# felipemcoelho/nf4-triton-dequantization

Hardware: AMD Instinct MI355X
Metric: dequantized elements/s (4096x4096 NF4->bf16, blocksize 64 / nested 256) (higher is better)
Workload: dtype f32

## Files before the change

nf4_triton_dequantization_amd/csrc/nf4_dequant.hip:

```cpp
#include <hip/hip_runtime.h>
#include <stdint.h>

#include <type_traits>

#include "../../include/nf4_dequant.h"
#include "nf4_common.h"
#include "nf4_dequant_plan.h"

namespace {

using namespace nf4dq;

#if NF4_FLAT_STAMPS
#define NF4_FSTAMP(slot_, val_)                                                                      \
    do {                                                                                             \
        __builtin_amdgcn_sched_barrier(0);                                                           \
        if (lane == 0) stamps[(blockIdx.x * kFlatWaves + (threadIdx.x >> 6)) * 4u + (slot_)] = (val_);    \
        __builtin_amdgcn_sched_barrier(0);                                                           \
    } while (0)
#define NF4_FNOW() __builtin_amdgcn_s_memrealtime()
#else
#define NF4_FSTAMP(slot_, val_) \
    do {                        \
    } while (0)
#define NF4_FNOW() 0ull
#endif

#ifndef NF4_DQ_AUX_STORE
#define NF4_DQ_AUX_STORE 18
#endif
#ifndef NF4_DQ_AUX_LOAD
#define NF4_DQ_AUX_LOAD 2
#endif
#ifndef NF4_DQ_SCALE_FIRST
#define NF4_DQ_SCALE_FIRST 0
#endif
#ifndef NF4_DQ_SCALE_NT
#define NF4_DQ_SCALE_NT 0
#endif
#ifndef NF4_DQ_DECODE
#define NF4_DQ_DECODE 1
#endif
#ifndef NF4_DQ_SINGLE_FAST
#define NF4_DQ_SINGLE_FAST 1
#endif
#ifndef NF4_DQ_ABL_NOSCALE
#define NF4_DQ_ABL_NOSCALE 0
#endif

constexpr int kAuxStore = NF4_DQ_AUX_STORE;
constexpr int kAuxLoad = NF4_DQ_AUX_LOAD;

struct TileIn {
    uint32_t w[kU];
    uint32_t a1;
    float a2;
};

template <int DT>
__device__ __forceinline__ uint32_t tile_block(const Desc& D, uint32_t base, uint32_t lane) {
    constexpr uint32_t kTileBytes = tile_bytes<DT>();
    const uint32_t bsh = D.blk_shift;
    const uint32_t bpt = kTileBytes >> bsh;
    uint32_t g = (base >> bsh) + (bpt ? (lane & (bpt - 1u)) : 0u);
    const uint32_t nblk = (D.nbytes + (1u << bsh) - 1u) >> bsh;
    g = g < nblk ? g : nblk - 1u;
    return g + D.blk_base;
}

template <int DT, int MODE, bool FENCE = false>
__device__ __forceinline__ TileIn tile_load(const Desc& D, __amdgpu_buffer_rsrc_t rp, uint32_t base, uint32_t lane) {
    constexpr uint32_t LB = lane_bytes<DT>();
    TileIn in;
    auto packed_loads = [&]() {
#pragma unroll
        for (int j = 0; j < kU; ++j) {
            const uint32_t off = base + 64u * LB * j + LB * lane;
            if constexpr (LB == 4) {
                in.w[j] = __builtin_amdgcn_raw_buffer_load_b32(rp, off, 0, kAuxLoad);
            } else {
                in.w[j] = __builtin_amdgcn_raw_buffer_load_b16(rp, off, 0, kAuxLoad);
            }
        }
    };
    if constexpr (!NF4_DQ_SCALE_FIRST) {
        packed_loads();
        if constexpr (FENCE) __builtin_amdgcn_sched_barrier(0);
    }
    const uint32_t g = tile_block<DT>(D, base, lane);
    if constexpr (NF4_DQ_ABL_NOSCALE) {
        in.a1 = g & 255u;
        in.a2 = 0.01f;
    } else if constexpr (MODE == kRef) {
        const uint32_t r = fdiv(g, D.bpr);
        const uint32_t b = g - r * D.bpr.d;
        const uint8_t* pa1 = D.a1 + fmodu(g, D.nb);
        const float* pa2 = D.a2 + fmodu(r * D.groups + (b >> 2), D.n2);
        if constexpr (NF4_DQ_SCALE_NT) {
            in.a1 = __builtin_nontemporal_load(pa1);
            in.a2 = __builtin_nontemporal_load(pa2);
        } else {
            in.a1 = *pa1;
            in.a2 = *pa2;
        }
    } else if constexpr (MODE == kSingle) {
        const uint32_t r = fdiv(g, D.bpr);
        const uint32_t b = g - r * D.bpr.d;
        in.a2 = D.a2[r * D.n2.d + b];
    } else if constexpr (MODE == kBnb) {
        in.a1 = D.a1[g];
        in.a2 = D.a2[g >> D.blk2_shift];
    } else {
        in.a2 = D.a2[g];
    }
    if constexpr (NF4_DQ_SCALE_FIRST) packed_loads();
    return in;
}

template <int DT, int MODE>
__device__ __forceinline__ void tile_finish(const Desc& D, __amdgpu_buffer_rsrc_t ro, const float* lut,
                                            const TileIn& in, uint32_t base, uint32_t lane, const float* code2s) {
    float s;
    if constexpr (MODE == kRef) {
        s = ((float)in.a1 / 127.0f) * in.a2;
    } else if constexpr (MODE == kBnb) {
        s = code2s[in.a1] * in.a2 + D.offset;
    } else {
        s = in.a2;
    }
    const uint32_t bsh = D.blk_shift;
    constexpr uint32_t kOB = out_bytes_per_packed_byte<DT>();
    constexpr uint32_t LB = lane_bytes<DT>();
#pragma unroll
    for (int j = 0; j < kU; ++j) {
        const uint32_t rel = 64u * LB * j + LB * lane;
        const float sj = __shfl(s, (int)(rel >> bsh), 64);
        const uint32_t w = in.w[j];
        const uint32_t hi4 = (w >> 2) & 0x3C3C3C3Cu;
        const uint32_t lo4 = (w << 2) & 0x3C3C3C3Cu;
        const char* t = reinterpret_cast<const char*>(lut);
        float v[2 * LB];
#pragma unroll
        for (int k = 0; k < (int)LB; ++k) {
            v[2 * k] = *reinterpret_cast<const float*>(t + ((hi4 >> (8 * k)) & 0xFFu)) * sj;
            v[2 * k + 1] = *reinterpret_cast<const float*>(t + ((lo4 >> (8 * k)) & 0xFFu)) * sj;
        }
        const uint32_t ob = (base + rel) * kOB;
        if constexpr (DT == NF4DQ_F32) {
            u32x4 o = {__float_as_uint(v[0]), __float_as_uint(v[1]), __float_as_uint(v[2]), __float_as_uint(v[3])};
            __builtin_amdgcn_raw_buffer_store_b128(o, ro, ob, 0, kAuxStore);
        } else {
            u32x4 o = {pack2<DT>(v[0], v[1]), pack2<DT>(v[2], v[3]), pack2<DT>(v[4], v[5]), pack2<DT>(v[6], v[7])};
            __builtin_amdgcn_raw_buffer_store_b128(o, ro, ob, 0, kAuxStore);
        }
    }
}


struct TblCtx {
    char* tbl;
    uint32_t tb;
    f32x2 c01;
};

template <int DT, int MODE>
__device__ __forceinline__ void tile_finish_tbl(const Desc& D, __amdgpu_buffer_rsrc_t ro, const TileIn& in,
                                                uint32_t base, uint32_t lane, const float* code2s,
                                                const TblCtx& c) {
    float s;
    if constexpr (MODE == kRef) {
        s = ((float)in.a1 / 127.0f) * in.a2;
    } else if constexpr (MODE == kBnb) {
        s = code2s[in.a1] * in.a2 + D.offset;
    } else {
        s = in.a2;
    }
    const uint32_t bsh = D.blk_shift;
    const uint32_t k = lane & 7u;
#pragma unroll
    for (int j = 0; j < kU; ++j) {
        const uint32_t rel = 256u * j + 4u * lane;
        const float sj = __shfl(s, (int)(rel >> bsh), 64);
        block_table_write<DT>(c.tbl, c.tb, k, c.c01, sj);
        const u32x4 ov = block_table_decode(c.tbl, c.tb, in.w[j]);
        __builtin_amdgcn_raw_buffer_store_b128(ov, ro, (base + rel) * 4u, 0, kAuxStore);
    }
}

template <int MAXB>
__device__ __forceinline__ uint32_t find_matrix(const Batch<MAXB>& bt, uint32_t t, uint32_t k) {
    if constexpr (MAXB > 1) {
        while (k + 1 < bt.count && t >= bt.d[k + 1].tile_begin) ++k;
    }
    return k;
}

struct Cursor {
    uint32_t t, k, base;
    bool valid;
};

template <int DT, int MAXB>
__device__ __forceinline__ Cursor cursor_at(const Batch<MAXB>& bt, uint32_t t, uint32_t k_hint) {
    constexpr uint32_t kTileBytes = tile_bytes<DT>();
    Cursor c;
    c.t = t;
    c.valid = t < bt.total_tiles;
    c.k = c.valid ? find_matrix(bt, t, k_hint) : k_hint;
    c.base = c.valid ? (t - bt.d[c.k].tile_begin) * kTileBytes : 0xFFFFF000u;
    return c;
}

template <int DT, int MAXB>
__device__ __forceinline__ void make_rsrcs(const Batch<MAXB>& bt, uint32_t k, __amdgpu_buffer_rsrc_t& rp,
                                           __amdgpu_buffer_rsrc_t& ro) {
    constexpr uint32_t kOB = out_bytes_per_packed_byte<DT>();
    rp = __builtin_amdgcn_make_buffer_rsrc((void*)bt.d[k].packed, 0, bt.d[k].nbytes, kRsrcFlags);
    ro = __builtin_amdgcn_make_buffer_rsrc((void*)bt.d[k].out, 0, bt.d[k].nbytes * kOB, kRsrcFlags);
}

template <int DT, int MODE, int MAXB>
__global__ __launch_bounds__(kFlatWg) void nf4_flat_kernel(const Batch<MAXB> bt) {
    __shared__ __attribute__((aligned(16))) float lut[16];
    __shared__ __attribute__((aligned(16))) float code2s[MODE == kBnb ? 256 : 1];
    constexpr bool kTbl = NF4_DQ_DECODE == 1 && DT != NF4DQ_F32;
    __shared__ __attribute__((aligned(256))) char tbl[kTbl ? kFlatWaves * 2048 : 4];
    const uint32_t lane = threadIdx.x & 63u;
#if NF4_FLAT_STAMPS
    const unsigned long long t_entry = NF4_FNOW();
    unsigned long long tiles_done = 0;
    unsigned long long* const stamps = bt.stamps;
#endif
    const uint32_t t0 = __builtin_amdgcn_readfirstlane(blockIdx.x * kFlatWaves + (threadIdx.x >> 6));
    const uint32_t nwaves = gridDim.x * kFlatWaves;

    float c2w = 0.0f;
    if constexpr (MODE == kBnb) c2w = bt.d[0].code2[threadIdx.x & 255u];
    Cursor ca = cursor_at<DT>(bt, t0, 0u);
    __amdgpu_buffer_rsrc_t rpa, roa;
    make_rsrcs<DT>(bt, ca.k, rpa, roa);
    TileIn A = tile_load<DT, MODE>(bt.d[ca.k], rpa, ca.base, lane);
    const bool multi = !NF4_DQ_SINGLE_FAST || ca.t + nwaves < bt.total_tiles;
    if (multi) {
        const u32x4 z = {0u, 0u, 0u, 0u};
#pragma unroll
        for (int j = 0; j < kU; ++j) __builtin_amdgcn_raw_buffer_store_b128(z, roa, 0xFFFFF000u + 16u * j, 0, kAuxStore);
    }
    write_lut(lut);
    if constexpr (MODE == kBnb) {
        if constexpr (kFlatWg >= 256) {
            if (threadIdx.x < 256u) code2s[threadIdx.x] = c2w;
        } else {
            for (uint32_t i = threadIdx.x; i < 256u; i += kFlatWg) code2s[i] = bt.d[0].code2[i];
        }
    }
    __syncthreads();
    TblCtx tc{};
    if constexpr (kTbl) {
        tc.tbl = tbl;
        tc.tb = ((threadIdx.x >> 6) << 11) + ((lane >> 3) << 8);
        tc.c01 = *reinterpret_cast<const f32x2*>(lut + 2u * (lane & 7u));
    }
    if (!ca.valid) {
        NF4_FSTAMP(0, t_entry);
        NF4_FSTAMP(1, 0ull);
        NF4_FSTAMP(2, NF4_FNOW());
        NF4_FSTAMP(3, 0ull);
        return;
    }
    if (!multi) {
        if constexpr (kTbl) tile_finish_tbl<DT, MODE>(bt.d[ca.k], roa, A, ca.base, lane, code2s, tc);
        else tile_finish<DT, MODE>(bt.d[ca.k], roa, lut, A, ca.base, lane, code2s);
#if NF4_FLAT_STAMPS
        NF4_FSTAMP(1, NF4_FNOW());
        __builtin_amdgcn_s_waitcnt(0);
        NF4_FSTAMP(0, t_entry);
        NF4_FSTAMP(2, NF4_FNOW());
        NF4_FSTAMP(3, 1ull);
#endif
        return;
    }
    while (true) {
        const Cursor cb = cursor_at<DT>(bt, ca.t + nwaves, ca.k);
        __amdgpu_buffer_rsrc_t rpb = rpa, rob = roa;
        if (MAXB > 1 && cb.k != ca.k) make_rsrcs<DT>(bt, cb.k, rpb, rob);
        TileIn B = tile_load<DT, MODE>(bt.d[cb.k], rpb, cb.base, lane);
        if constexpr (kTbl) tile_finish_tbl<DT, MODE>(bt.d[ca.k], roa, A, ca.base, lane, code2s, tc);
        else tile_finish<DT, MODE>(bt.d[ca.k], roa, lut, A, ca.base, lane, code2s);
#if NF4_FLAT_STAMPS
        if (tiles_done == 0) NF4_FSTAMP(1, NF4_FNOW());
        ++tiles_done;
#endif
        if (!cb.valid) break;

        const Cursor cn = cursor_at<DT>(bt, cb.t + nwaves, cb.k);
        __amdgpu_buffer_rsrc_t rpn = rpb, ron = rob;
        if (MAXB > 1 && cn.k != cb.k) make_rsrcs<DT>(bt, cn.k, rpn, ron);
        A = tile_load<DT, MODE>(bt.d[cn.k], rpn, cn.base, lane);
        if constexpr (kTbl) tile_finish_tbl<DT, MODE>(bt.d[cb.k], rob, B, cb.base, lane, code2s, tc);
        else tile_finish<DT, MODE>(bt.d[cb.k], rob, lut, B, cb.base, lane, code2s);
#if NF4_FLAT_STAMPS
        ++tiles_done;
#endif
        if (!cn.valid) break;
        ca = cn;
        rpa = rpn;
        roa = ron;
    }
#if NF4_FLAT_STAMPS
    __builtin_amdgcn_s_waitcnt(0);
    NF4_FSTAMP(0, t_entry);
    NF4_FSTAMP(2, NF4_FNOW());
    NF4_FSTAMP(3, tiles_done);
#endif
}

template <int DT, int MODE>
__global__ __launch_bounds__(kFlatWg) void nf4_flat1_kernel(
    const uint32_t* packed, uint32_t nbytes, uint32_t tiles, u32x4* out,
    const uint8_t* a1, const float* a2, uint32_t blk_shift, uint32_t blk_base, uint32_t groups, uint32_t bpr_d,
    uint32_t bpr_mul, uint32_t bpr_shift, uint32_t nb_d, uint32_t nb_mul, uint32_t nb_shift, uint32_t n2_d,
    uint32_t n2_mul, uint32_t n2_shift, const float* code2, float offset, uint32_t blk2_shift
#if NF4_FLAT_STAMPS
    , unsigned long long* stamps
#endif
) {
    __shared__ __attribute__((aligned(16))) float lut[16];
    __shared__ __attribute__((aligned(16))) float code2s[MODE == kBnb ? 256 : 1];
    constexpr bool kTbl = NF4_DQ_DECODE == 1 && DT != NF4DQ_F32;
    __shared__ __attribute__((aligned(256))) char tbl[kTbl ? kFlatWaves * 2048 : 4];
    const uint32_t lane = threadIdx.x & 63u;
#if NF4_FLAT_STAMPS
    const unsigned long long t_entry = NF4_FNOW();
#endif
    const uint32_t t0 = __builtin_amdgcn_readfirstlane(blockIdx.x * kFlatWaves + (threadIdx.x >> 6));
    const bool valid = t0 < tiles;
    const uint32_t base = valid ? t0 * tile_bytes<DT>() : 0xFFFFF000u;
    Desc D;
    D.packed = packed;
    D.a1 = a1;
    D.a2 = a2;
    D.code2 = code2;
    D.out = out;
    D.offset = offset;
    D.nbytes = nbytes;
    D.tile_begin = 0u;
    D.groups = groups;
    D.nb = FastDiv{nb_d, nb_mul, nb_shift};
    D.n2 = FastDiv{n2_d, n2_mul, n2_shift};
    D.bpr = FastDiv{bpr_d, bpr_mul, bpr_shift};
    D.blk_shift = blk_shift;
    D.blk2_shift = blk2_shift;
    D.blk_base = blk_base;
    const __amdgpu_buffer_rsrc_t rp = __builtin_amdgcn_make_buffer_rsrc((void*)packed, 0, nbytes, kRsrcFlags);
    const __amdgpu_buffer_rsrc_t ro =
        __builtin_amdgcn_make_buffer_rsrc((void*)out, 0, nbytes * out_bytes_per_packed_byte<DT>(), kRsrcFlags);
    const TileIn A = tile_load<DT, MODE, true>(D, rp, base, lane);
    write_lut(lut);
    if constexpr (MODE == kBnb) {
        for (uint32_t i = threadIdx.x; i < 256u; i += kFlatWg) code2s[i] = code2[i];
    }
    __syncthreads();
    if (!valid) {
        NF4_FSTAMP(0, t_entry);
        NF4_FSTAMP(1, 0ull);
        NF4_FSTAMP(2, NF4_FNOW());
        NF4_FSTAMP(3, 0ull);
        return;
    }
    if constexpr (kTbl) {
        TblCtx tc;
        tc.tbl = tbl;
        tc.tb = ((threadIdx.x >> 6) << 11) + ((lane >> 3) << 8);
        tc.c01 = *reinterpret_cast<const f32x2*>(lut + 2u * (lane & 7u));
        tile_finish_tbl<DT, MODE>(D, ro, A, base, lane, code2s, tc);
    } else {
        tile_finish<DT, MODE>(D, ro, lut, A, base, lane, code2s);
    }
#if NF4_FLAT_STAMPS
    NF4_FSTAMP(1, NF4_FNOW());
    __builtin_amdgcn_s_waitcnt(0);
    NF4_FSTAMP(0, t_entry);
    NF4_FSTAMP(2, NF4_FNOW());
    NF4_FSTAMP(3, 1ull);
#endif
}

template <int DT, int MODE>
__global__ __launch_bounds__(kWg) void nf4_rows_kernel(const RowsArgs A) {
    __shared__ __attribute__((aligned(16))) float lut[16];
    write_lut(lut);
    __syncthreads();
    const int64_t total = A.m * A.cols_b;
    for (int64_t i = (int64_t)blockIdx.x * kWg + threadIdx.x; i < total; i += (int64_t)gridDim.x * kWg) {
        const int64_t r = i / A.cols_b;
        const int64_t j = i - r * A.cols_b;
        const int64_t b = j >> 5;
        float s;
        if constexpr (MODE == kRef) {
            const float q = (float)A.a1[(r * A.bpr + b) % A.nb];
            s = (q / 127.0f) * A.a2[(r * A.groups + (b >> 2)) % A.n2];
        } else {
            s = A.a2[r * A.rs + b];
        }
        const uint32_t byte = A.packed[r * A.stride + j];
        const int64_t c = 2 * j;
        store1<DT>(A.out, r * A.n + c, lut[byte >> 4] * s);
        if (c + 1 < A.n) store1<DT>(A.out, r * A.n + c + 1, lut[byte & 15u] * s);
    }
}


constexpr uint32_t kDrop = 0xFFFFFFF0u;
constexpr int kAuxPiece = 0;
constexpr uint32_t kStageBytes = 4128;
constexpr uint32_t kStageDummy = 4112;

inline __device__ uint32_t range32(uint64_t v) { return v > 0x7FFFFFFFull ? 0x7FFFFFFFu : (uint32_t)v; }

inline __device__ uint32_t opaque_mul(uint32_t a, uint32_t b) {
    uint32_t r = a * b;
    asm("" : "+v"(r));
    return r;
}

template <int DT>
__device__ __forceinline__ void chunk_table_build(char* ctbl, uint32_t region, uint32_t lane, float sb) {
    uint32_t e[8];
#pragma unroll
    for (int k = 0; k < 8; ++k)
        e[k] = pack2<DT>(__uint_as_float(kNf4Bits[2 * k]) * sb, __uint_as_float(kNf4Bits[2 * k + 1]) * sb);
    u32x4_alias* dst = reinterpret_cast<u32x4_alias*>(ctbl + region + 32u * lane);
    dst[0] = u32x4{e[0], e[1], e[2], e[3]};
    dst[1] = u32x4{e[4], e[5], e[6], e[7]};
}

__device__ __forceinline__ void chunk_table_decode(const char* ctbl, uint32_t region, uint32_t w, uint32_t t,
                                                   uint32_t (&p)[4]) {
    t &= 63u;
    const uint32_t base = region + ((t >> 3) << 8);
    const uint32_t rep = __builtin_amdgcn_perm(0u, (t & 7u) << 5, 0x00000000u);
    const uint32_t hb = ((w >> 3) & 0x1E1E1E1Eu) | rep;
    const uint32_t lb = ((w << 1) & 0x1E1E1E1Eu) | rep;
#pragma unroll
    for (int b = 0; b < 4; ++b) {
        const uint32_t ah = __builtin_amdgcn_perm(hb, base, 0x03020104u + b);
        const uint32_t al = __builtin_amdgcn_perm(lb, base, 0x03020104u + b);
        const uint32_t vh = *reinterpret_cast<const u16_alias*>(ctbl + ah);
        const uint32_t vl = *reinterpret_cast<const u16_alias*>(ctbl + al);
        p[b] = vh | (vl << 16);
    }
}

template <int DT, int MODE>
__global__ __launch_bounds__(kWg) void nf4_chunk_dense_kernel(const ChunkArgs A) {
    __shared__ __attribute__((aligned(256))) char ctbl[4 * 2048];
    const uint32_t lane = threadIdx.x & 63u;
    const uint32_t cw = __builtin_amdgcn_readfirstlane((blockIdx.x * 4u + (threadIdx.x >> 6)) * 256u);
    const __amdgpu_buffer_rsrc_t rp =
        __builtin_amdgcn_make_buffer_rsrc((void*)A.packed, 0, (uint32_t)A.packed_len, kRsrcFlags);
    const __amdgpu_buffer_rsrc_t ro =
        __builtin_amdgcn_make_buffer_rsrc(A.out, 0, (uint32_t)(A.out_elems * 2u), kRsrcFlags);
    uint32_t w[4];
#pragma unroll
    for (int j = 0; j < 4; ++j)
        w[j] = __builtin_amdgcn_raw_buffer_load_b32(rp, 4u * (cw + 64u * j + lane), 0, kAuxLoad);
    __builtin_amdgcn_sched_barrier(0);
    const uint32_t cw0 = min(cw, A.chunks - 1u);
    const uint32_t r0 = fdiv(cw0, A.L);
    const uint32_t q0 = cw0 - r0 * A.L.d;
    const uint32_t cl = min(cw + 255u, A.chunks - 1u);
    const uint32_t rl = fdiv(cl, A.L);
    const uint32_t g0 = r0 * A.bpr.d + (q0 >> 3);
    const uint32_t gl = rl * A.bpr.d + ((cl - rl * A.L.d) >> 3);
    float sb;
    {
        const uint32_t g = min(g0 + lane, gl);
        const uint32_t r = fdiv(g, A.bpr);
        const uint32_t b = g - r * A.bpr.d;
        if constexpr (MODE == kRef) {
            const float q8 = (float)A.a1[fmodu(g, A.nb)];
            sb = (q8 / 127.0f) * A.a2[fmodu(opaque_mul(r, A.groups) + (b >> 2), A.n2)];
        } else {
            sb = A.a2[opaque_mul(r, A.rs) + b];
        }
    }
    uint32_t gsel[4];
    {
        uint32_t q = q0 + lane;
        const bool wrap = q >= A.L.d;
        q = wrap ? q - A.L.d : q;
        uint32_t gr = (wrap ? A.bpr.d : 0u) + r0 * A.bpr.d - g0;
#pragma unroll
        for (int j = 0; j < 4; ++j) {
            if (j) {
                q += 64u;
                const bool wj = q >= A.L.d;
                q = wj ? q - A.L.d : q;
                gr += wj ? A.bpr.d : 0u;
            }
            gsel[j] = gr + (q >> 3);
        }
    }
    const uint32_t region = (threadIdx.x >> 6) << 11;
    chunk_table_build<DT>(ctbl, region, lane, sb);
#pragma unroll
    for (int j = 0; j < 4; ++j) {
        uint32_t p[4];
        chunk_table_decode(ctbl, region, w[j], gsel[j], p);
        const u32x4 o = {p[0], p[1], p[2], p[3]};
        __builtin_amdgcn_raw_buffer_store_b128(o, ro, 16u * (cw + 64u * j + lane), 0, kAuxStore);
    }
}

template <int DT, int MODE, int LW, int SW>
__global__ __launch_bounds__(kWg) void nf4_chunk_kernel(const ChunkArgs A) {
    __shared__ __attribute__((aligned(16))) float lut[16];
    __shared__ __attribute__((aligned(256))) char ctbl[DT == NF4DQ_F32 ? 4 : 4 * 2048];
    __shared__ __attribute__((aligned(16))) char stage[DT != NF4DQ_F32 && SW != 16 ? 4 * kStageBytes : 16];
    constexpr uint32_t kOB = DT == NF4DQ_F32 ? 4u : 2u;
    const uint32_t lane = threadIdx.x & 63u;
    const uint32_t cw = __builtin_amdgcn_readfirstlane((blockIdx.x * 4u + (threadIdx.x >> 6)) * 256u);
    const uint32_t cw0 = min(cw, A.chunks - 1u);
    const uint32_t r0 = fdiv(cw0, A.L);
    const uint32_t q0 = cw0 - r0 * A.L.d;
    const uint64_t pb = (uint64_t)r0 * A.stride;
    const uintptr_t pw = (uintptr_t)(A.packed + pb);
    const uint32_t kb = LW == 4 ? 0u : (uint32_t)(pw & 3u);
    const uint64_t plen = LW == 4 ? A.packed_len - pb : ((A.packed_len - pb + kb + 3u) & ~uint64_t(3));
    const __amdgpu_buffer_rsrc_t rp =
        __builtin_amdgcn_make_buffer_rsrc((void*)(pw - kb), 0, range32(plen), kRsrcFlags);
    auto load_chunk = [&](uint32_t po) -> uint32_t {
        if constexpr (LW == 4) {
            return __builtin_amdgcn_raw_buffer_load_b32(rp, po, 0, 0);
        } else {
            const uint32_t a = po == kDrop ? kDrop : po + kb;
            const uint32_t lo = __builtin_amdgcn_raw_buffer_load_b32(rp, a & ~3u, 0, 0);
            const uint32_t hi = __builtin_amdgcn_raw_buffer_load_b32(rp, (a & ~3u) + 4u, 0, 0);
            return __builtin_amdgcn_alignbyte(hi, lo, a & 3u);
        }
    };
    const uint32_t g0 = r0 * A.bpr.d + (q0 >> 3);
    uint32_t gl = 0;
    bool shared = false;
    auto span_blocks = [&]() {
        const uint32_t cl = min(cw + 255u, A.chunks - 1u);
        const uint32_t rl = fdiv(cl, A.L);
        gl = rl * A.bpr.d + ((cl - rl * A.L.d) >> 3);
        shared = gl - g0 < 64u;
    };
    uint32_t w[4], rel[4], col[4], gsel[4];
    float s[4] = {0.0f, 0.0f, 0.0f, 0.0f};
    uint32_t ga1 = 0;
    float ga2 = 0.0f;
    auto gather = [&]() {
        if (shared) {
            const uint32_t g = min(g0 + lane, gl);
            const uint32_t r = fdiv(g, A.bpr);
            const uint32_t b = g - r * A.bpr.d;
            if constexpr (MODE == kRef) {
                ga1 = A.a1[fmodu(g, A.nb)];
                ga2 = A.a2[fmodu(opaque_mul(r, A.groups) + (b >> 2), A.n2)];
            } else {
                ga2 = A.a2[opaque_mul(r, A.rs) + b];
            }
        }
    };
    if (A.L.d >= 64u) {
        uint32_t qj[4], dr[4];
        {
            uint32_t q = q0 + lane, d = 0, pr = 0;
#pragma unroll
            for (int j = 0; j < 4; ++j) {
                if (j) q += 64u;
                const bool wrap = q >= A.L.d;
                q = wrap ? q - A.L.d : q;
                d += wrap ? 1u : 0u;
                pr += wrap ? A.stride : 0u;
                qj[j] = q;
                dr[j] = d;
                w[j] = load_chunk(cw + 64u * j + lane < A.chunks ? pr + 4u * q : kDrop);
            }
        }
        __builtin_amdgcn_sched_barrier(0);
#pragma unroll
        for (int j = 0; j < 4; ++j) {
            const bool ok = cw + 64u * j + lane < A.chunks;
            col[j] = ok ? 8u * qj[j] : 0x7FFFFFF0u;
            rel[j] = dr[j] * A.n + 8u * qj[j] - 8u * q0;
            gsel[j] = dr[j] * A.bpr.d + (qj[j] >> 3) - (q0 >> 3);
        }
    } else {
        uint32_t po[4], pa1[4], pa2[4];
#pragma unroll
        for (int j = 0; j < 4; ++j) {
            const uint32_t c = cw + 64u * j + lane;
            const bool ok = c < A.chunks;
            const uint32_t r = ok ? fdiv(c, A.L) : r0;
            const uint32_t q = ok ? c - r * A.L.d : q0;
            po[j] = ok ? (r - r0) * A.stride + 4u * q : kDrop;
            col[j] = ok ? 8u * q : 0x7FFFFFF0u;
            rel[j] = (r - r0) * A.n + 8u * q - 8u * q0;
            gsel[j] = r * A.bpr.d + (q >> 3) - g0;
            const uint32_t b = q >> 3;
            if constexpr (MODE == kRef) {
                pa1[j] = fmodu(r * A.bpr.d + b, A.nb);
                pa2[j] = fmodu(opaque_mul(r, A.groups) + (b >> 2), A.n2);
            } else {
                pa1[j] = 0;
                pa2[j] = opaque_mul(r, A.rs) + b;
            }
        }
#pragma unroll
        for (int j = 0; j < 4; ++j) w[j] = load_chunk(po[j]);
        __builtin_amdgcn_sched_barrier(0);
        span_blocks();
        if (!shared) {
#pragma unroll
            for (int j = 0; j < 4; ++j) {
                if constexpr (MODE == kRef) s[j] = ((float)A.a1[pa1[j]] / 127.0f) * A.a2[pa2[j]];
                else s[j] = A.a2[pa2[j]];
            }
        }
    }
    if (A.L.d >= 64u) span_blocks();
    gather();
    const uint64_t e0 = (uint64_t)r0 * A.n + 8ull * q0;
    const __amdgpu_buffer_rsrc_t ro = __builtin_amdgcn_make_buffer_rsrc(
        (void*)((char*)A.out + e0 * kOB), 0, range32((A.out_elems - e0) * kOB), kRsrcFlags);
    float sb = 0.0f;
    if constexpr (MODE == kRef) sb = ((float)ga1 / 127.0f) * ga2;
    else sb = ga2;
    const uint32_t sbase = (threadIdx.x >> 6) * kStageBytes;
    const uint32_t sa = (uint32_t)(((uintptr_t)A.out >> 1) + e0) & 7u;
    auto store16 = [&](int j, const uint32_t (&p)[4]) {
        if constexpr (SW == 16) {
            const u32x4 o = {p[0], p[1], p[2], p[3]};
            __builtin_amdgcn_raw_buffer_store_b128(o, ro, col[j] < A.n ? rel[j] * 2u : kDrop, 0, kAuxStore);
        } else {
            const bool ok = cw + 64u * (uint32_t)j + lane < A.chunks;
            char* a = stage + sbase + (ok ? 2u * (rel[j] + sa) : kStageDummy);
#pragma unroll
            for (int i = 7; i >= 0; --i) {
                reinterpret_cast<u16_alias*>(a)[i] = (uint16_t)(p[i >> 1] >> (16 * (i & 1)));
                asm volatile("" ::: "memory");
            }
        }
    };
    uint32_t span = 0;
    uintptr_t ob = 0, l_first = 0, l_last = 0;
    if constexpr (SW != 16) {
        const uint32_t cl2 = min(cw + 255u, A.chunks - 1u);
        const uint32_t rl2 = fdiv(cl2, A.L);
        const uint32_t ql2 = cl2 - rl2 * A.L.d;
        span = cw >= A.chunks ? 0u : (uint32_t)((uint64_t)rl2 * A.n + min(8u * ql2 + 8u, A.n) - e0);
        ob = (uintptr_t)A.out + 2u * e0;
        l_first = ob >> 7;
        l_last = (ob + 2u * span - 1u) >> 7;
    }
    auto store_pieces = [&](uint32_t k0, uint32_t k1) {
        for (uint32_t kb = k0; kb < k1; kb += 64u) {
            const uint32_t k = kb + lane;
            const int x0 = (int)(8u * k) - (int)sa;
            const bool whole = k < k1 && x0 >= 0 && x0 + 8 <= (int)span;
            const u32x4 v = *reinterpret_cast<const u32x4_alias*>(stage + sbase + 16u * (k < k1 ? k : k0));
            const uint32_t off = whole ? 2u * (uint32_t)x0 : kDrop;
            const uintptr_t l = (ob + 2u * (uint32_t)x0) >> 7;
            if (l == l_first || l == l_last) __builtin_amdgcn_raw_buffer_store_b128(v, ro, off, 0, kAuxPiece);
            else __builtin_amdgcn_raw_buffer_store_b128(v, ro, off, 0, kAuxStore);
        }
    };
    auto flush_step = [&](int j, uint32_t& kdone) {
        if constexpr (SW != 16) {
            const uint32_t rel63 = __builtin_amdgcn_readlane(rel[j], 63);
            const uint32_t col63 = __builtin_amdgcn_readlane(col[j], 63);
            const uint32_t e_end = col63 < A.n ? rel63 + min(8u, A.n - col63) : span;
            const uint32_t kmax = (e_end + sa) >> 3;
            store_pieces(kdone, kmax);
            kdone = kmax > kdone ? kmax : kdone;
        }
    };
    auto flush16 = [&](uint32_t kdone) {
        if constexpr (SW != 16) {
            if (cw >= A.chunks) return;
            store_pieces(kdone, (span + sa) >> 3);
            const __amdgpu_buffer_rsrc_t rsp =
                __builtin_amdgcn_make_buffer_rsrc((void*)((char*)A.out + e0 * 2u), 0, 2u * span, kRsrcFlags);
            const uint32_t klast = (span + sa - 1u) >> 3;
            const uint32_t k = lane == 0u ? 0u : klast;
            const int xe = (int)(8u * k) - (int)sa;
            if (lane < 2u && (lane == 0u || klast != 0u) && !(xe >= 0 && xe + 8 <= (int)span)) {
                const u32x4 v = *reinterpret_cast<const u32x4_alias*>(stage + sbase + 16u * k);
#pragma unroll
                for (int i = 0; i < 8; ++i)
                    __builtin_amdgcn_raw_buffer_store_b16((uint16_t)(v[i >> 1] >> (16 * (i & 1))), rsp,
                                                          2u * (uint32_t)(xe + i), 0, kAuxPiece);
            }
        }
    };
    if constexpr (DT != NF4DQ_F32) {
        if (A.L.d >= 64u) {
            const uint32_t region = (threadIdx.x >> 6) << 11;
            chunk_table_build<DT>(ctbl, region, lane, sb);
            uint32_t kdone = 0;
#pragma unroll
            for (int j = 0; j < 4; ++j) {
                uint32_t p[4];
                chunk_table_decode(ctbl, region, w[j], gsel[j], p);
                store16(j, p);
                if (j < 3 && cw < A.chunks) flush_step(j, kdone);
            }
            flush16(kdone);
            return;
        }
    }
    write_lut(lut);
    __syncthreads();
    const char* t = reinterpret_cast<const char*>(lut);
#pragma unroll
    for (int j = 0; j < 4; ++j) {
        const uint32_t hi4 = (w[j] >> 2) & 0x3C3C3C3Cu;
        const uint32_t lo4 = (w[j] << 2) & 0x3C3C3C3Cu;
        const float sh = __shfl(sb, (int)gsel[j], 64);
        const float sj = shared ? sh : s[j];
        float v[8];
#pragma unroll
        for (int k = 0; k < 4; ++k) {
            v[2 * k] = *reinterpret_cast<const float*>(t + ((hi4 >> (8 * k)) & 0xFFu)) * sj;
            v[2 * k + 1] = *reinterpret_cast<const float*>(t + ((lo4 >> (8 * k)) & 0xFFu)) * sj;
        }
        if constexpr (DT == NF4DQ_F32) {
            const uint32_t ob = rel[j] * 4u;
            if constexpr (SW == 16) {
#pragma unroll
                for (int h = 0; h < 2; ++h) {
                    const u32x4 o = {__float_as_uint(v[4 * h]), __float_as_uint(v[4 * h + 1]),
                                     __float_as_uint(v[4 * h + 2]), __float_as_uint(v[4 * h + 3])};
                    __builtin_amdgcn_raw_buffer_store_b128(o, ro, col[j] + 4u * h < A.n ? ob + 16u * h : kDrop, 0,
                                                           kAuxPiece);
                }
            } else {
#pragma unroll
                for (int i = 0; i < 8; ++i)
                    __builtin_amdgcn_raw_buffer_store_b32(__float_as_uint(v[i]), ro, col[j] + i < A.n ? ob + 4u * i : kDrop,
                                                          0, kAuxPiece);
            }
        } else {
            uint32_t p[4];
#pragma unroll
            for (int k = 0; k < 4; ++k) p[k] = pack2<DT>(v[2 * k], v[2 * k + 1]);
            store16(j, p);
        }
    }
    if constexpr (DT != NF4DQ_F32) flush16(0u);
}


constexpr uint32_t kPieceTbl = 4096;

__device__ __forceinline__ uint32_t bytes4(uint32_t x) { return __builtin_amdgcn_perm(0u, x, 0u); }

template <uint32_t EP, int RE>
struct PieceWave {
    int32_t fw;
    uint32_t c0, g0, gl;
    int32_t c[4], b[4];
    uint32_t gr[4], lo[4], hi[4];
    uint32_t nb[4], lo2[4], hi2[4];
};

template <uint32_t EP, int RE>
__device__ __forceinline__ bool piece_wave(const PieceArgs& A, uint32_t kw, uint32_t lane, PieceWave<EP, RE>& W) {
    if (EP * kw >= A.sa + A.elems) return false;
    W.fw = (int32_t)(EP * kw) - (int32_t)A.sa;
    const uint32_t fwc = W.fw < 0 ? 0u : (uint32_t)W.fw;
    const uint32_t r0 = fdiv(fwc, A.nf);
    W.c0 = fwc - r0 * A.nf.d;
    const __amdgpu_buffer_rsrc_t rp = __builtin_amdgcn_make_buffer_rsrc((void*)A.packed, 0, A.prange, kRsrcFlags);
    uint32_t aj[4], an[4];
    {
        int32_t c = (W.fw < 0 ? W.fw : (int32_t)W.c0) + (int32_t)(EP * lane);
        uint32_t pb = A.kb + r0 * A.stride;
        uint32_t gb = 0u - (W.c0 >> 6);
#pragma unroll
        for (int j = 0; j < 4; ++j) {
            if (j) c += (int32_t)(64u * EP);
            const bool wrap = c >= (int32_t)A.n;
            c = wrap ? c - (int32_t)A.n : c;
            pb = wrap ? pb + A.stride : pb;
            gb = wrap ? gb + A.bpr.d : gb;
            W.c[j] = c;
            W.gr[j] = gb;
            W.b[j] = (int32_t)pb + (c >> 1);
            aj[j] = (uint32_t)(W.b[j] & ~3);
            if constexpr (RE == 2) {
                W.nb[j] = pb + A.stride;
                an[j] = c > (int32_t)(A.n - EP) ? W.nb[j] & ~3u : kDrop;
            } else {
                W.nb[j] = W.lo2[j] = W.hi2[j] = 0u;
                an[j] = 0u;
            }
        }
    }
#pragma unroll
    for (int j = 0; j < 4; ++j) {
        uint32_t a4 = aj[j] + 4u;
        asm("" : "+v"(a4));
        W.lo[j] = __builtin_amdgcn_raw_buffer_load_b32(rp, aj[j], 0, 0);
        W.hi[j] = __builtin_amdgcn_raw_buffer_load_b32(rp, a4, 0, 0);
        if constexpr (RE == 2) {
            uint32_t n4 = an[j] + 4u;
            asm("" : "+v"(n4));
            W.lo2[j] = __builtin_amdgcn_raw_buffer_load_b32(rp, an[j], 0, 0);
            W.hi2[j] = __builtin_amdgcn_raw_buffer_load_b32(rp, n4, 0, 0);
        }
    }
    __builtin_amdgcn_sched_barrier(0);
    W.g0 = r0 * A.bpr.d + (W.c0 >> 6);
    const uint32_t fl = min((uint32_t)(W.fw + (int32_t)(256u * EP) - 1), A.elems - 1u);
    const uint32_t rl = fdiv(fl, A.nf);
    W.gl = rl * A.bpr.d + ((fl - rl * A.nf.d) >> 6);
    return true;
}

template <int MODE>
__device__ __forceinline__ float piece_scale(const PieceArgs& A, uint32_t g0, uint32_t gl, uint32_t lane) {
    const uint32_t g = min(g0 + lane, gl);
    const uint32_t r = fdiv(g, A.bpr);
    const uint32_t b = g - r * A.bpr.d;
    if constexpr (MODE == kRef) {
        const float q8 = (float)A.a1[fmodu(g, A.nb)];
        return (q8 / 127.0f) * A.a2[fmodu(opaque_mul(r, A.groups) + (b >> 2), A.n2)];
    } else {
        return A.a2[opaque_mul(r, A.rs) + b];
    }
}

template <int SH, int RE, bool TRI>
__device__ __forceinline__ void piece_codes(uint32_t lo, uint32_t hi, int32_t b, int32_t c, uint32_t ib_in,
                                            uint32_t ib_end, uint32_t slot, uint32_t lo2, uint32_t hi2,
                                            uint32_t nb, uint32_t& es, uint32_t& os) {
    constexpr uint32_t kCode = 0x0F0F0F0Fu << SH, kStep = 0x01010101u << (SH + 4), kEP = 16u >> SH;
    auto yE = [](uint32_t ib) { return ((0x86848280u - bytes4(ib)) >> (3 - SH)) & kStep; };
    auto yO = [](uint32_t ib) { return ((0x87858381u - bytes4(ib)) >> (3 - SH)) & kStep; };
    uint32_t sE, sO, eE, eO;
    if constexpr (TRI) {
        eE = yE(ib_end);
        eO = yO(ib_end);
        sE = eE + yE(ib_in);
        sO = eO + yO(ib_in);
    } else {
        sE = yE(min(ib_in, ib_end));
        sO = yO(min(ib_in, ib_end));
        eE = ib_end < kEP ? sE : 0u;
        eO = ib_end < kEP ? sO : 0u;
    }
    const uint32_t sel = bytes4((uint32_t)b & 3u) + 0x03020100u;
    const uint32_t w0 = __builtin_amdgcn_perm(hi, lo, sel);
    const uint32_t w1 = __builtin_amdgcn_perm(hi, lo, sel + 0x01010101u);
    const uint32_t h0 = __builtin_amdgcn_alignbit(w0, w0, 4u - SH);
    const uint32_t l0 = __builtin_amdgcn_alignbit(w0, w0, 32u - SH);
    const uint32_t h1 = __builtin_amdgcn_alignbit(w1, w1, 4u - SH);
    const bool odd = (c & 1) != 0;
    uint32_t E = odd ? l0 : h0, O = odd ? h1 : l0;
    if constexpr (RE != 0) {
        uint32_t E2, O2;
        if constexpr (RE == 1) {
            const uint32_t l1 = __builtin_amdgcn_alignbit(w1, w1, 32u - SH);
            E2 = O;
            O2 = odd ? l1 : h1;
        } else {
            const uint32_t wn = __builtin_amdgcn_perm(hi2, lo2, bytes4(nb & 3u) + 0x03020100u);
            const uint32_t hn = __builtin_amdgcn_alignbit(wn, wn, 4u - SH);
            const uint32_t ln = __builtin_amdgcn_alignbit(wn, wn, 32u - SH);
            const uint32_t e = ib_end, eodd = e & 1u;
            E2 = (eodd ? ln : hn) << ((8u * ((e + 1u) >> 1)) & 31u);
            O2 = (eodd ? hn : ln) << ((8u * (e >> 1)) & 31u);
        }
        const uint32_t kE = eE - (eE >> 4);
        const uint32_t kO = eO - (eO >> 4);
        E = (E2 & kE) | (E & ~kE);
        O = (O2 & kO) | (O & ~kO);
    }
    const uint32_t rep = bytes4(slot << (SH + 4));
    es = (E & kCode) | (rep + sE);
    os = (O & kCode) | (rep + sO);
}

template <int DT, int MODE, int RE, bool TRI>
__global__ __launch_bounds__(kWg) void nf4_piece_kernel(const PieceArgs A) {
    __shared__ __attribute__((aligned(256))) char ptbl[4 * kPieceTbl];
    const uint32_t lane = threadIdx.x & 63u;
    const uint32_t kw = __builtin_amdgcn_readfirstlane((blockIdx.x * 4u + (threadIdx.x >> 6)) * 256u);
    PieceWave<8, RE> W;
    if (!piece_wave<8, RE>(A, kw, lane, W)) return;
    const float sb = piece_scale<MODE>(A, W.g0, W.gl, lane);
    const uint32_t region = (threadIdx.x >> 6) * kPieceTbl;
    {
        uint32_t e[8];
#pragma unroll
        for (int k = 0; k < 8; ++k)
            e[k] = pack2<DT>(__uint_as_float(kNf4Bits[2 * k]) * sb, __uint_as_float(kNf4Bits[2 * k + 1]) * sb);
        u32x4_alias* d0 = reinterpret_cast<u32x4_alias*>(ptbl + region + ((lane >> 2) << 8) + ((lane & 3u) << 5));
        d0[0] = u32x4{e[0], e[1], e[2], e[3]};
        d0[1] = u32x4{e[4], e[5], e[6], e[7]};
        if (lane >= 4u) {
            u32x4_alias* d1 = reinterpret_cast<u32x4_alias*>(ptbl + region + ((lane >> 2) << 8) - 256u + 128u +
                                                            ((lane & 3u) << 5));
            d1[0] = u32x4{e[0], e[1], e[2], e[3]};
            d1[1] = u32x4{e[4], e[5], e[6], e[7]};
        }
    }
    const __amdgpu_buffer_rsrc_t ro =
        __builtin_amdgcn_make_buffer_rsrc(A.line, 0, 2u * (A.sa + A.elems), kRsrcFlags);
#pragma unroll
    for (int j = 0; j < 4; ++j) {
        const uint32_t cu = (uint32_t)max(W.c[j], 0);
        const uint32_t tA = min(W.gr[j] + (cu >> 6), 59u);
        const uint32_t to_blk = 64u - (cu & 63u), to_end = A.n - cu;
        const uint32_t ib_in = to_blk < to_end ? min(to_blk, 8u) : 8u, ib_end = min(to_end, 8u);
        uint32_t es, os;
        piece_codes<1, RE, TRI>(W.lo[j], W.hi[j], W.b[j], W.c[j], ib_in, ib_end, tA & 3u, W.lo2[j], W.hi2[j],
                                W.nb[j], es, os);
        const uint32_t base = region + ((tA >> 2) << 8);
        uint32_t p[4];
#pragma unroll
        for (int b = 0; b < 4; ++b) {
            const uint32_t ve = *reinterpret_cast<const u16_alias*>(ptbl + __builtin_amdgcn_perm(es, base, 0x03020104u + b));
            const uint32_t vo = *reinterpret_cast<const u16_alias*>(ptbl + __builtin_amdgcn_perm(os, base, 0x03020104u + b));
            p[b] = __builtin_amdgcn_perm(vo, ve, 0x05040100u);
        }
        const uint32_t k = kw + 64u * (uint32_t)j + lane;
        const int32_t f = W.fw + 8 * (64 * j + (int32_t)lane);
        const bool whole = f >= 0 && (uint32_t)f + 8u <= A.elems;
        const u32x4 o = {p[0], p[1], p[2], p[3]};
        __builtin_amdgcn_raw_buffer_store_b128(o, ro, whole ? 16u * k : kDrop, 0, kAuxStore);
        if (!whole && f < (int32_t)A.elems && f + 8 > 0) {
            const __amdgpu_buffer_rsrc_t rsp =
                __builtin_amdgcn_make_buffer_rsrc(A.out, 0, 2u * A.elems, kRsrcFlags);
#pragma unroll
            for (int i = 0; i < 8; ++i) {
                uint32_t oe = 2u * (uint32_t)(f + i);
                asm("" : "+v"(oe));
                __builtin_amdgcn_raw_buffer_store_b16((uint16_t)(p[i >> 1] >> (16 * (i & 1))), rsp, oe, 0,
                                                      kAuxPiece);
            }
        }
    }
}

constexpr uint32_t kPiece32Tbl = 12 * 256;

template <int MODE, int RE, bool TRI>
__global__ __launch_bounds__(kWg) void nf4_piece32_kernel(const PieceArgs A) {
    __shared__ __attribute__((aligned(256))) char ptbl[4 * kPiece32Tbl];
    const uint32_t lane = threadIdx.x & 63u;
    const uint32_t kw = __builtin_amdgcn_readfirstlane((blockIdx.x * 4u + (threadIdx.x >> 6)) * 256u);
    PieceWave<4, RE> W;
    if (!piece_wave<4, RE>(A, kw, lane, W)) return;
    const float sb = piece_scale<MODE>(A, W.g0, W.gl, lane);
    const uint32_t region = (threadIdx.x >> 6) * kPiece32Tbl;
    if (lane < 24u) {
        u32x4 e[4];
#pragma unroll
        for (int k = 0; k < 4; ++k)
            e[k] = u32x4{__float_as_uint(__uint_as_float(kNf4Bits[4 * k]) * sb),
                         __float_as_uint(__uint_as_float(kNf4Bits[4 * k + 1]) * sb),
                         __float_as_uint(__uint_as_float(kNf4Bits[4 * k + 2]) * sb),
                         __float_as_uint(__uint_as_float(kNf4Bits[4 * k + 3]) * sb)};
        u32x4_alias* d0 = reinterpret_cast<u32x4_alias*>(ptbl + region + ((lane >> 1) << 8) + ((lane & 1u) << 6));
#pragma unroll
        for (int k = 0; k < 4; ++k) d0[k] = e[k];
        if (lane >= 2u) {
            u32x4_alias* d1 = reinterpret_cast<u32x4_alias*>(ptbl + region + ((lane >> 1) << 8) - 256u + 128u +
                                                            ((lane & 1u) << 6));
#pragma unroll
            for (int k = 0; k < 4; ++k) d1[k] = e[k];
        }
    }
    const __amdgpu_buffer_rsrc_t ro =
        __builtin_amdgcn_make_buffer_rsrc(A.line, 0, 4u * (A.sa + A.elems), kRsrcFlags);
#pragma unroll
    for (int j = 0; j < 4; ++j) {
        const uint32_t cu = (uint32_t)max(W.c[j], 0);
        const uint32_t tA = min(W.gr[j] + (cu >> 6), 21u);
        const uint32_t to_blk = 64u - (cu & 63u), to_end = A.n - cu;
        const uint32_t ib_in = to_blk < to_end ? min(to_blk, 4u) : 4u, ib_end = min(to_end, 4u);
        uint32_t es, os;
        piece_codes<2, RE, TRI>(W.lo[j], W.hi[j], W.b[j], W.c[j], ib_in, ib_end, tA & 1u, W.lo2[j], W.hi2[j],
                                W.nb[j], es, os);
        const uint32_t base = region + ((tA >> 1) << 8);
        uint32_t p[4];
#pragma unroll
        for (int b = 0; b < 2; ++b) {
            p[2 * b] = *reinterpret_cast<const uint32_t*>(ptbl + __builtin_amdgcn_perm(es, base, 0x03020104u + b));
            p[2 * b + 1] = *reinterpret_cast<const uint32_t*>(ptbl + __builtin_amdgcn_perm(os, base, 0x03020104u + b));
        }
        const uint32_t k = kw + 64u * (uint32_t)j + lane;
        const int32_t f = W.fw + 4 * (64 * j + (int32_t)lane);
        const bool whole = f >= 0 && (uint32_t)f + 4u <= A.elems;
        const u32x4 o = {p[0], p[1], p[2], p[3]};
        __builtin_amdgcn_raw_buffer_store_b128(o, ro, whole ? 16u * k : kDrop, 0, kAuxStore);
        if (!whole && f < (int32_t)A.elems && f + 4 > 0) {
            const __amdgpu_buffer_rsrc_t rsp =
                __builtin_amdgcn_make_buffer_rsrc(A.out, 0, 4u * A.elems, kRsrcFlags);
#pragma unroll
            for (int i = 0; i < 4; ++i) {
                uint32_t oe = 4u * (uint32_t)(f + i);
                asm("" : "+v"(oe));
                __builtin_amdgcn_raw_buffer_store_b32(p[i], rsp, oe, 0, kAuxPiece);
            }
        }
    }
}

template <int DT>
__global__ __launch_bounds__(kWg) void nf4_bnb_bytes_kernel(const BnbBytesArgs A) {
    __shared__ __attribute__((aligned(16))) float lut[16];
    write_lut(lut);
    __syncthreads();
    const int64_t nbytes = (A.numel + 1) / 2;
    for (int64_t i = (int64_t)blockIdx.x * kWg + threadIdx.x; i < nbytes; i += (int64_t)gridDim.x * kWg) {
        const int64_t e = 2 * i;
        const int64_t blk = e >> A.blk_shift_elems;
        const float s = A.single ? A.a2[blk] : A.code2[A.a1[blk]] * A.a2[blk >> A.blk2_shift] + A.offset;
        const uint32_t byte = A.packed[i];
        store1<DT>(A.out, e, lut[byte >> 4] * s);
        if (e + 1 < A.numel) store1<DT>(A.out, e + 1, lut[byte & 15u] * s);
    }
}

inline int hip_rc(hipError_t e) { return e == hipSuccess ? NF4DQ_OK : NF4DQ_ERR_HIP_BASE + (int)e; }

#if NF4_FLAT_STAMPS
unsigned long long* g_stamps = nullptr;
#endif

int cu_count() {
    int dev = 0, cus = 0;
    if (hipGetDevice(&dev) != hipSuccess) return 256;
    if (hipDeviceGetAttribute(&cus, hipDeviceAttributeMultiprocessorCount, dev) != hipSuccess || cus <= 0) return 256;
    return cus;
}

template <int V0, int... Vs, class F>
void with_const(int v, F&& f) {
    if constexpr (sizeof...(Vs) == 0) f(std::integral_constant<int, V0>{});
    else if (v == V0) f(std::integral_constant<int, V0>{});
    else with_const<Vs...>(v, f);
}

template <int DT, int MODE, int MAXB>
void run_flat(const Launch& L, hipStream_t st) {
#if NF4_FLAT_STAMPS
    Batch<MAXB> b = L.as<Batch<MAXB>>();
    b.stamps = g_stamps;
#else
    const Batch<MAXB>& b = L.as<Batch<MAXB>>();
#endif
    if constexpr (MAXB == 1 && NF4_DQ_FLAT1) {
        if (L.family == kFlat1) {
            const Desc& d = b.d[0];
            nf4_flat1_kernel<DT, MODE><<<dim3(L.grid), dim3(L.block), 0, st>>>(
                d.packed, d.nbytes, b.total_tiles, reinterpret_cast<u32x4*>(d.out), d.a1, d.a2, d.blk_shift,
                d.blk_base, d.groups, d.bpr.d, d.bpr.mul, d.bpr.shift, d.nb.d, d.nb.mul, d.nb.shift, d.n2.d, d.n2.mul,
                d.n2.shift, d.code2, d.offset, d.blk2_shift
#if NF4_FLAT_STAMPS
                , b.stamps
#endif
            );
            return;
        }
    }
    hipLaunchKernelGGL((nf4_flat_kernel<DT, MODE, MAXB>), dim3(L.grid), dim3(L.block), 0, st, b);
}

int run(const Launch& L, hipStream_t st) {
    const dim3 g(L.grid), blk(L.block);
    with_const<NF4DQ_BF16, NF4DQ_F16, NF4DQ_F32>(L.dtype, [&](auto dt) {
        constexpr int DT = decltype(dt)::value;
        if (L.family == kFlat1 || L.family == kFlat) {
            with_const<kRef, kSingle, kBnb, kBnbSingle>(L.mode, [&](auto md) {
                if (L.p0 == 1) run_flat<DT, decltype(md)::value, 1>(L, st);
                else run_flat<DT, decltype(md)::value, NF4DQ_BATCH_MAX>(L, st);
            });
        } else if (L.family == kBnbBytes) {
            hipLaunchKernelGGL((nf4_bnb_bytes_kernel<DT>), g, blk, 0, st, L.as<BnbBytesArgs>());
        } else {
            with_const<kRef, kSingle>(L.mode, [&](auto md) {
                constexpr int MODE = decltype(md)::value;
                if (L.family == kRows) {
                    hipLaunchKernelGGL((nf4_rows_kernel<DT, MODE>), g, blk, 0, st, L.as<RowsArgs>());
                } else if (L.family == kChunkDense) {
                    if constexpr (DT != NF4DQ_F32)
                        hipLaunchKernelGGL((nf4_chunk_dense_kernel<DT, MODE>), g, blk, 0, st, L.as<ChunkArgs>());
                } else if (L.family == kChunk) {
                    with_const<4, 1>(L.p0, [&](auto lw) {
                        with_const<16, 4>(L.p1, [&](auto sw) {
                            hipLaunchKernelGGL((nf4_chunk_kernel<DT, MODE, decltype(lw)::value, decltype(sw)::value>), g,
                                               blk, 0, st, L.as<ChunkArgs>());
                        });
                    });
                } else {
                    with_const<2, 1, 0>(L.p0, [&](auto re) {
                        with_const<1, 0>(L.p1, [&](auto tri) {
                            constexpr int RE = decltype(re)::value;
                            constexpr bool TRI = decltype(tri)::value != 0;
                            if constexpr (DT == NF4DQ_F32)
                                hipLaunchKernelGGL((nf4_piece32_kernel<MODE, RE, TRI>), g, blk, 0, st, L.as<PieceArgs>());
                            else
                                hipLaunchKernelGGL((nf4_piece_kernel<DT, MODE, RE, TRI>), g, blk, 0, st,
                                                   L.as<PieceArgs>());
                        });
                    });
                }
            });
        }
    });
    return hip_rc(hipGetLastError());
}

struct OnStream {
    hipStream_t st;
    int operator()(const Launch& L) const { return run(L, st); }
};

}

extern "C" {

int nf4_dequant_ref(const uint8_t* packed, int64_t packed_len, const uint8_t* absmax_q, int64_t nb,
                    const float* absmax2, int64_t n2, void* out, int32_t out_dtype, int64_t m, int64_t n,
                    void* hip_stream) {
    OnStream emit{reinterpret_cast<hipStream_t>(hip_stream)};
    return plan_ref(packed, packed_len, absmax_q, nb, absmax2, n2, out, out_dtype, m, n, kDefaultCfg, 0, emit);
}

int nf4_dequant_ref_cfg(const uint8_t* packed, int64_t packed_len, const uint8_t* absmax_q, int64_t nb,
                        const float* absmax2, int64_t n2, void* out, int32_t out_dtype, int64_t m, int64_t n,
                        const nf4_launch_cfg* cfg, void* hip_stream) {
    OnStream emit{reinterpret_cast<hipStream_t>(hip_stream)};
    nf4_launch_cfg c;
    if (const int rc = check_cfg(cfg, c)) return rc;
    return plan_ref(packed, packed_len, absmax_q, nb, absmax2, n2, out, out_dtype, m, n, c,
                    c.blocks_per_cu > 0 ? cu_count() : 0, emit);
}

int nf4_dequant_single(const uint8_t* packed, int64_t packed_len, const float* absmax, int64_t absmax_len,
                       void* out, int32_t out_dtype, int64_t m, int64_t n, void* hip_stream) {
    OnStream emit{reinterpret_cast<hipStream_t>(hip_stream)};
    return plan_single(packed, packed_len, absmax, absmax_len, out, out_dtype, m, n, emit);
}

int nf4_dequant_ref_batched(const nf4_matrix_desc* descs, int32_t count, int32_t out_dtype, void* hip_stream) {
    OnStream emit{reinterpret_cast<hipStream_t>(hip_stream)};
    return plan_ref_batched(descs, count, out_dtype, emit);
}

int nf4_dequant_bnb(const uint8_t* packed, const uint8_t* absmax_q, int64_t nb, const float* code2,
                    const float* absmax2, int64_t n2, float offset, void* out, int32_t out_dtype, int64_t numel,
                    int32_t blocksize, int32_t blocksize2, void* hip_stream) {
    OnStream emit{reinterpret_cast<hipStream_t>(hip_stream)};
    return plan_bnb(packed, absmax_q, nb, code2, absmax2, n2, offset, out, out_dtype, numel, blocksize, blocksize2,
                    false, emit);
}

int nf4_dequant_bnb_single(const uint8_t* packed, const float* absmax, int64_t nabs, void* out, int32_t out_dtype,
                           int64_t numel, int32_t blocksize, void* hip_stream) {
    OnStream emit{reinterpret_cast<hipStream_t>(hip_stream)};
    return plan_bnb(packed, nullptr, nabs, nullptr, absmax, 0, 0.0f, out, out_dtype, numel, blocksize, 1, true, emit);
}

const char* nf4_strerror(int code) {
    switch (code) {
        case NF4DQ_OK: return "ok";
        case NF4DQ_ERR_ARG: return "invalid argument (null pointer, dtype or negative size)";
        case NF4DQ_ERR_SHAPE: return "shape mismatch (packed weight / absmax cannot be viewed as the reference does)";
        case NF4DQ_ERR_TOO_LARGE: return "matrix too large for one launch";
        case NF4DQ_ERR_SPLITK_TIMEOUT:
            return "fused GEMM split-K hand-off timed out (some outputs are NaN; workspace re-zeroed)";
        default: break;
    }
    if (code >= NF4DQ_ERR_HIP_BASE) return hipGetErrorString((hipError_t)(code - NF4DQ_ERR_HIP_BASE));
    return "unknown error";
}

const char* nf4_version(void) { return "nf4dq 0.2.0 gfx950"; }

#if NF4_FLAT_STAMPS
void nf4_dbg_set_stamps(void* buf) { g_stamps = reinterpret_cast<unsigned long long*>(buf); }
#endif

}
```

Baseline: 2335 billion.

## Prefetch a later wave's packed tile into L2 via buffer-load-to-LDS

After finishing its own tile, each wave in the single-tile path issues a buffer load into LDS of the packed bytes of the tile kPfTiles ahead. The intent is to warm the XCD-local L2 for the wave that will later own that tile, which is why the stride is a multiple of 8 times the waves per workgroup. The LDS data is discarded, so the cost is extra loads issued per wave, a small amount of extra LDS, and a possible delay to wave exit. The chosen distance suits this matrix size and may not fit other shapes.

Result: no change. 2323 billion (-0.5%).

```diff
diff --git a/nf4_triton_dequantization_amd/csrc/nf4_dequant.hip b/nf4_triton_dequantization_amd/csrc/nf4_dequant.hip
--- a/nf4_triton_dequantization_amd/csrc/nf4_dequant.hip
+++ b/nf4_triton_dequantization_amd/csrc/nf4_dequant.hip
@@ -46,6 +46,12 @@
 #endif
 #ifndef NF4_DQ_ABL_NOSCALE
 #define NF4_DQ_ABL_NOSCALE 0
+#endif
+#ifndef NF4_DQ_PREFETCH_TILES
+#define NF4_DQ_PREFETCH_TILES 20480
+#endif
+#ifndef NF4_DQ_AUX_PREFETCH
+#define NF4_DQ_AUX_PREFETCH 16
 #endif
 
 constexpr int kAuxStore = NF4_DQ_AUX_STORE;
@@ -117,6 +123,32 @@
     return in;
 }
 
+constexpr uint32_t kPfTiles = NF4_DQ_PREFETCH_TILES;
+constexpr int kAuxPf = NF4_DQ_AUX_PREFETCH;
+static_assert(kPfTiles % (8u * kFlatWaves) == 0, "the prefetching workgroup must share its XCD with the tile's owner");
+
+template <int DT>
+constexpr uint32_t pf_line_bytes() { return tile_bytes<DT>() % 1024u == 0 ? 1024u : 256u; }
+
+template <int DT>
+__device__ __forceinline__ void tile_prefetch(__amdgpu_buffer_rsrc_t rp, uint32_t base, uint32_t lane, char* line) {
+    constexpr uint32_t kTileBytes = tile_bytes<DT>();
+    static_assert(kTileBytes % 256u == 0, "a tile is whole 256-byte wave loads");
+    __builtin_amdgcn_sched_barrier(0);
+    const uint32_t pb = base + kPfTiles * kTileBytes;
+    __attribute__((address_space(3))) void* dst = (__attribute__((address_space(3))) void*)line;
+    if constexpr (kTileBytes % 1024u == 0) {
+#pragma unroll
+        for (uint32_t j = 0; j < kTileBytes / 1024u; ++j)
+            __builtin_amdgcn_raw_ptr_buffer_load_lds(rp, dst, 16, pb + 1024u * j + 16u * lane, 0, 0, kAuxPf);
+    } else {
+#pragma unroll
+        for (uint32_t j = 0; j < kTileBytes / 256u; ++j)
+            __builtin_amdgcn_raw_ptr_buffer_load_lds(rp, dst, 4, pb + 256u * j + 4u * lane, 0, 0, kAuxPf);
+    }
+    __builtin_amdgcn_sched_barrier(0);
+}
+
 template <int DT, int MODE>
 __device__ __forceinline__ void tile_finish(const Desc& D, __amdgpu_buffer_rsrc_t ro, const float* lut,
                                             const TileIn& in, uint32_t base, uint32_t lane, const float* code2s) {
@@ -225,6 +257,7 @@
     __shared__ __attribute__((aligned(16))) float code2s[MODE == kBnb ? 256 : 1];
     constexpr bool kTbl = NF4_DQ_DECODE == 1 && DT != NF4DQ_F32;
     __shared__ __attribute__((aligned(256))) char tbl[kTbl ? kFlatWaves * 2048 : 4];
+    __shared__ __attribute__((aligned(16))) char pfl[kPfTiles ? kFlatWaves * pf_line_bytes<DT>() : 4];
     const uint32_t lane = threadIdx.x & 63u;
 #if NF4_FLAT_STAMPS
     const unsigned long long t_entry = NF4_FNOW();
@@ -239,6 +272,9 @@
     Cursor ca = cursor_at<DT>(bt, t0, 0u);
     __amdgpu_buffer_rsrc_t rpa, roa;
     make_rsrcs<DT>(bt, ca.k, rpa, roa);
+    constexpr uint32_t kPfBytes = kPfTiles * tile_bytes<DT>();
+    const uint32_t nby = bt.d[ca.k].nbytes;
+    const bool pf = kPfTiles != 0 && nby > kPfBytes && ca.base < nby - kPfBytes;
     TileIn A = tile_load<DT, MODE>(bt.d[ca.k], rpa, ca.base, lane);
     const bool multi = !NF4_DQ_SINGLE_FAST || ca.t + nwaves < bt.total_tiles;
     if (multi) {
@@ -273,6 +309,11 @@
         else tile_finish<DT, MODE>(bt.d[ca.k], roa, lut, A, ca.base, lane, code2s);
 #if NF4_FLAT_STAMPS
         NF4_FSTAMP(1, NF4_FNOW());
+#endif
+        if constexpr (kPfTiles != 0) {
+            if (pf) tile_prefetch<DT>(rpa, ca.base, lane, pfl + __builtin_amdgcn_readfirstlane(threadIdx.x >> 6) * pf_line_bytes<DT>());
+        }
+#if NF4_FLAT_STAMPS
         __builtin_amdgcn_s_waitcnt(0);
         NF4_FSTAMP(0, t_entry);
         NF4_FSTAMP(2, NF4_FNOW());
@@ -329,6 +370,7 @@
     __shared__ __attribute__((aligned(16))) float code2s[MODE == kBnb ? 256 : 1];
     constexpr bool kTbl = NF4_DQ_DECODE == 1 && DT != NF4DQ_F32;
     __shared__ __attribute__((aligned(256))) char tbl[kTbl ? kFlatWaves * 2048 : 4];
+    __shared__ __attribute__((aligned(16))) char pfl[kPfTiles ? kFlatWaves * pf_line_bytes<DT>() : 4];
     const uint32_t lane = threadIdx.x & 63u;
 #if NF4_FLAT_STAMPS
     const unsigned long long t_entry = NF4_FNOW();
@@ -379,6 +421,12 @@
     }
 #if NF4_FLAT_STAMPS
     NF4_FSTAMP(1, NF4_FNOW());
+#endif
+    if constexpr (kPfTiles != 0) {
+        if (t0 + kPfTiles < tiles)
+            tile_prefetch<DT>(rp, base, lane, pfl + __builtin_amdgcn_readfirstlane(threadIdx.x >> 6) * pf_line_bytes<DT>());
+    }
+#if NF4_FLAT_STAMPS
     __builtin_amdgcn_s_waitcnt(0);
     NF4_FSTAMP(0, t_entry);
     NF4_FSTAMP(2, NF4_FNOW());
```
